# theislab/dca

Measured on NVIDIA H100. Metric: cells/sec (ZINB AE epoch, device-timed), higher is better.
Workload: dtype bf16-gemm/f32-acc/f32-loss

## Files before the change

### dca_b200/csrc/dense_tc.cu

```cuda
#include <mutex>
#include "engine.h"
#include "tc_common.cuh"
#include "head_act.cuh"

namespace dca {
namespace tc {

typedef CUresult (*EncodeTiledFn)(CUtensorMap*, CUtensorMapDataType, cuuint32_t, void*, const cuuint64_t*,
                                  const cuuint64_t*, const cuuint32_t*, const cuuint32_t*, CUtensorMapInterleave,
                                  CUtensorMapSwizzle, CUtensorMapL2promotion, CUtensorMapFloatOOBfill);

static EncodeTiledFn encode_fn() {
  static EncodeTiledFn fn = nullptr;
  static std::once_flag once;
  std::call_once(once, [] {
    void* p = nullptr;
    cudaDriverEntryPointQueryResult q;
    if (cudaGetDriverEntryPoint("cuTensorMapEncodeTiled", &p, cudaEnableDefault, &q) == cudaSuccess &&
        q == cudaDriverEntryPointSuccess)
      fn = reinterpret_cast<EncodeTiledFn>(p);
  });
  return fn;
}

int make_tensor_map_2d(CUtensorMap* out, const void* base, int elem_bytes, int is_bf16, uint64_t rows, uint64_t cols,
                       uint64_t ld_elems, uint32_t box_rows, uint32_t box_cols, int swizzle) {
  EncodeTiledFn fn = encode_fn();
  if (!fn) { set_error("cuTensorMapEncodeTiled is not available from the driver"); return DCA_ERR_CUDA; }
  cuuint64_t dims[2] = {cols, rows};
  cuuint64_t strides[1] = {ld_elems * (uint64_t)elem_bytes};
  cuuint32_t box[2] = {box_cols, box_rows};
  cuuint32_t estr[2] = {1, 1};
  const CUtensorMapDataType dt = is_bf16 ? CU_TENSOR_MAP_DATA_TYPE_BFLOAT16 : CU_TENSOR_MAP_DATA_TYPE_FLOAT32;
  CUresult r = fn(out, dt, 2, const_cast<void*>(base), dims, strides, box, estr, CU_TENSOR_MAP_INTERLEAVE_NONE,
                  swizzle ? CU_TENSOR_MAP_SWIZZLE_128B : CU_TENSOR_MAP_SWIZZLE_NONE, CU_TENSOR_MAP_L2_PROMOTION_L2_256B,
                  CU_TENSOR_MAP_FLOAT_OOB_FILL_NONE);
  if (r != CUDA_SUCCESS) {
    set_error("cuTensorMapEncodeTiled failed (%d): rows=%llu cols=%llu ld=%llu box=%ux%u elem=%d", (int)r,
              (unsigned long long)rows, (unsigned long long)cols, (unsigned long long)ld_elems, box_rows, box_cols, elem_bytes);
    return DCA_ERR_CUDA;
  }
  return DCA_OK;
}

struct ProbeParams {
  int a_mn, b_mn, M, N, K;
  int a_boxes, a_box_bytes, a_box_c0, a_box_c1;
  int b_boxes, b_box_bytes, b_box_c0, b_box_c1;
  uint32_t a_lbo, a_sbo, a_kstep, a_kblock_steps, a_kblock_bytes, a_mn64_bytes;
  uint32_t b_lbo, b_sbo, b_kstep, b_kblock_steps, b_kblock_bytes, b_mn64_bytes;
};

template <int NC, int TA, int TB>
__device__ __forceinline__ void probe_mma(float (&acc)[NC / 2], uint64_t da, uint64_t db) {
  if constexpr (NC == 128) wgmma_m64n128k16<TA, TB>(acc, da, db, 1u);
  else wgmma_m64n64k16<TA, TB>(acc, da, db, 1u);
}

template <int NC>
__device__ __forceinline__ void probe_chunk(const ProbeParams& p, uint32_t sa, uint32_t sb, int m0, int n0, float* D) {
  float acc[NC / 2];
#pragma unroll
  for (int i = 0; i < NC / 2; ++i) acc[i] = 0.f;
  const uint32_t a0 = sa + (uint32_t)(m0 / 64) * p.a_mn64_bytes, b0 = sb + (uint32_t)(n0 / 64) * p.b_mn64_bytes;
  wgmma_fence();
  for (int j = 0; j < p.K / 16; ++j) {
    const uint32_t aoff = (j / p.a_kblock_steps) * p.a_kblock_bytes + (j % p.a_kblock_steps) * p.a_kstep;
    const uint32_t boff = (j / p.b_kblock_steps) * p.b_kblock_bytes + (j % p.b_kblock_steps) * p.b_kstep;
    const uint64_t da = make_smem_desc(a0 + aoff, p.a_lbo, p.a_sbo), db = make_smem_desc(b0 + boff, p.b_lbo, p.b_sbo);
    if (p.a_mn) { if (p.b_mn) probe_mma<NC, 1, 1>(acc, da, db); else probe_mma<NC, 1, 0>(acc, da, db); }
    else        { if (p.b_mn) probe_mma<NC, 0, 1>(acc, da, db); else probe_mma<NC, 0, 0>(acc, da, db); }
  }
  wgmma_commit();
  wgmma_wait<0>();
  acc_fence(acc);
  const int w = threadIdx.x >> 5, l = threadIdx.x & 31;
#pragma unroll
  for (int i = 0; i < NC / 2; ++i) {
    const int row = m0 + 16 * w + (l >> 2) + 8 * ((i >> 1) & 1), col = n0 + 8 * (i >> 2) + 2 * (l & 3) + (i & 1);
    D[(size_t)row * p.N + col] = acc[i];
  }
}

__global__ void __launch_bounds__(128, 1)
tc_probe_kernel(const __grid_constant__ CUtensorMap map_a, const __grid_constant__ CUtensorMap map_b,
                const ProbeParams p, float* __restrict__ D) {
  extern __shared__ __align__(1024) uint8_t smem_raw[];
  uint8_t* smem = smem_raw + ((1024u - (smem_u32(smem_raw) & 1023u)) & 1023u);
  __shared__ uint64_t bar_load;
  uint8_t* sa = smem;
  uint8_t* sb = smem + (size_t)p.a_boxes * p.a_box_bytes;
  if (threadIdx.x == 0) { mbar_init(&bar_load, 1); fence_barrier_init(); }
  __syncthreads();
  if (threadIdx.x == 0) {
    mbar_expect_tx(&bar_load, (uint32_t)(p.a_boxes * p.a_box_bytes + p.b_boxes * p.b_box_bytes));
    for (int i = 0; i < p.a_boxes; ++i) tma_load_2d(sa + (size_t)i * p.a_box_bytes, &map_a, i * p.a_box_c0, i * p.a_box_c1, &bar_load);
    for (int i = 0; i < p.b_boxes; ++i) tma_load_2d(sb + (size_t)i * p.b_box_bytes, &map_b, i * p.b_box_c0, i * p.b_box_c1, &bar_load);
  }
  mbar_wait(&bar_load, 0);
  for (int m0 = 0; m0 < p.M; m0 += 64)
    for (int n0 = 0; n0 < p.N;) {
      if (p.N - n0 >= 128) { probe_chunk<128>(p, smem_u32(sa), smem_u32(sb), m0, n0, D); n0 += 128; }
      else { probe_chunk<64>(p, smem_u32(sa), smem_u32(sb), m0, n0, D); n0 += 64; }
    }
}

namespace k2 {
constexpr int BM = 128, BN = 128, BK = 64;
constexpr int kThreads = 256;
constexpr uint32_t kABytes = BM * BK * 2, kBBytes = BN * BK * 2;
constexpr uint32_t kSmemBytes = kABytes + kBBytes + 1024;

struct Params {
  int B, G, n_heads;
  int kind[3];
  int m_tiles, n_tiles_per_head;
  const float* bias[3];
  const float* row_scale;
  float* out[3]; int64_t ld_out;
};

__global__ void __launch_bounds__(kThreads, 2)
heads_fwd_kernel(const __grid_constant__ CUtensorMap map_h, const __grid_constant__ CUtensorMap map_w0,
                 const __grid_constant__ CUtensorMap map_w1, const __grid_constant__ CUtensorMap map_w2, const Params p) {
  extern __shared__ __align__(1024) uint8_t smem_raw[];
  uint8_t* smem = smem_raw + ((1024u - (smem_u32(smem_raw) & 1023u)) & 1023u);
  __shared__ uint64_t full_bar;
  const int mt = blockIdx.x % p.m_tiles, r = blockIdx.x / p.m_tiles;
  const int nt = r % p.n_tiles_per_head, hs = r / p.n_tiles_per_head;
  if (threadIdx.x == 0) {
    mbar_init(&full_bar, 1);
    fence_barrier_init();
    const CUtensorMap* mw = hs == 0 ? &map_w0 : (hs == 1 ? &map_w1 : &map_w2);
    mbar_expect_tx(&full_bar, kABytes + kBBytes);
    tma_load_2d(smem, &map_h, 0, mt * BM, &full_bar);
    tma_load_2d(smem + kABytes, mw, nt * BN, 0, &full_bar);
    tma_load_2d(smem + kABytes + kBBytes / 2, mw, nt * BN + 64, 0, &full_bar);
  }
  __syncthreads();
  const int wg = threadIdx.x >> 7, w = (threadIdx.x >> 5) & 3, l = threadIdx.x & 31;
  const int col0 = nt * BN + 2 * (l & 3);
  const int row0 = mt * BM + wg * 64 + 16 * w + (l >> 2);
  const float* bias = p.bias[hs];
  const int kind = p.kind[hs];
  float2 bz[16];
#pragma unroll
  for (int c = 0; c < 16; ++c) bz[c] = (col0 + 8 * c < p.G) ? *reinterpret_cast<const float2*>(bias + col0 + 8 * c) : make_float2(0.f, 0.f);
  float rs[2] = {1.f, 1.f};
  if (kind == EPI_MEAN_ACT && p.row_scale) {
    if (row0 < p.B) rs[0] = p.row_scale[row0];
    if (row0 + 8 < p.B) rs[1] = p.row_scale[row0 + 8];
  }
  float acc[64];
#pragma unroll
  for (int i = 0; i < 64; ++i) acc[i] = 0.f;
  mbar_wait(&full_bar, 0);
  head_tile_mma(acc, smem_u32(smem) + wg * 64 * 128, smem_u32(smem) + kABytes);
  float* out = p.out[hs];
  auto emit = [&](auto act) {
#pragma unroll
    for (int h = 0; h < 2; ++h) {
      const int row = row0 + 8 * h;
      if (row >= p.B) continue;
      float* orow = out + (int64_t)row * p.ld_out;
#pragma unroll
      for (int c = 0; c < 16; ++c) {
        const int col = col0 + 8 * c;
        if (col < p.G)
          *reinterpret_cast<float2*>(orow + col) =
              make_float2(act(acc[4 * c + 2 * h], bz[c].x, rs[h]), act(acc[4 * c + 2 * h + 1], bz[c].y, rs[h]));
      }
    }
  };
  if (kind == EPI_MEAN_ACT) emit([](float a, float b, float s) { return head_out<EPI_MEAN_ACT>(a, b, s); });
  else if (kind == EPI_DISP_ACT) emit([](float a, float b, float s) { return head_out<EPI_DISP_ACT>(a, b, s); });
  else emit([](float a, float b, float s) { return head_out<EPI_SIGMOID>(a, b, s); });
}
}

int heads_fwd_tc(const __nv_bfloat16* Hb, int B, const __nv_bfloat16* const W[3], const float* const bias[3], int G,
                 int n_heads, const int kind[3], const float* row_scale, float* const out[3], int64_t ld_out, int sm_count,
                 cudaStream_t s) {
  using namespace k2;
  if (ld_out % 4 != 0 || G % 8 != 0) { set_error("heads_fwd_tc: G must be a multiple of 8 and ld_out of 4 (TMA strides)"); return DCA_ERR_BAD_ARG; }
  CUtensorMap mh, mw[3];
  DCA_TRY(make_tensor_map_2d(&mh, Hb, 2, 1, (uint64_t)B, 64, 64, BM, BK, 1));
  for (int i = 0; i < 3; ++i)
    DCA_TRY(make_tensor_map_2d(&mw[i], W[i < n_heads ? i : 0], 2, 1, 64, (uint64_t)G, (uint64_t)G, 64, 64, 1));
  Params p;
  p.B = B; p.G = G; p.n_heads = n_heads;
  for (int i = 0; i < 3; ++i) { const int k = i < n_heads ? i : 0; p.kind[i] = kind[i]; p.bias[i] = bias[k]; p.out[i] = out[k]; }
  p.m_tiles = cdiv(B, BM); p.n_tiles_per_head = cdiv(G, BN);
  p.row_scale = row_scale; p.ld_out = ld_out;
  (void)sm_count;
  static bool attr_set = false;
  if (!attr_set) {
    DCA_CUDA_OK(cudaFuncSetAttribute(heads_fwd_kernel, cudaFuncAttributeMaxDynamicSharedMemorySize, (int)kSmemBytes));
    attr_set = true;
  }
  const int grid = p.m_tiles * p.n_tiles_per_head * n_heads;
  heads_fwd_kernel<<<grid, kThreads, kSmemBytes, s>>>(mh, mw[0], mw[1], mw[2], p);
  DCA_LAUNCH_CHECK();
  return DCA_OK;
}

}

Engine::~Engine() {
  comm_destroy();
  for (auto e : prof.ev) cudaEventDestroy(e);
  for (auto& g : graphs) if (g.exec) cudaGraphExecDestroy(g.exec);
  if (hs.copy) cudaStreamDestroy(hs.copy);
  if (hs.expand) cudaStreamDestroy(hs.expand);
  for (int k = 0; k < 3; ++k) {
    if (hs.ready[k]) cudaEventDestroy(hs.ready[k]);
    if (hs.step_done[k]) cudaEventDestroy(hs.step_done[k]);
  }
  for (int k = 0; k < 2; ++k) {
    if (hs.h2d_done[k]) cudaEventDestroy(hs.h2d_done[k]);
    if (hs.cnt_free[k]) cudaEventDestroy(hs.cnt_free[k]);
  }
}

}

using namespace dca;

extern "C" int dca_tc_probe(const void* A, int32_t a_rows, int32_t a_cols, const void* Bm, int32_t b_rows, int32_t b_cols,
                            int32_t a_mn_major, int32_t b_mn_major, int32_t M, int32_t N, int32_t K,
                            int32_t a_lbo, int32_t a_sbo, int32_t b_lbo, int32_t b_sbo, float* D, void* stream) {
  using namespace tc;
  if (M != 128 || N % 64 != 0 || N < 64 || N > 256 || K % 64 != 0 || K <= 0 || K > 256) {
    set_error("dca_tc_probe: need M=128, N%%64==0 (64..256), K%%64==0 (<=256)"); return DCA_ERR_BAD_ARG;
  }
  ProbeParams p{};
  p.a_mn = a_mn_major; p.b_mn = b_mn_major; p.M = M; p.N = N; p.K = K;
  CUtensorMap ma, mb;
  auto setup = [&](int mn, int mn_extent, int rows, int cols, const void* base, CUtensorMap* map, int& boxes, int& box_bytes,
                   int& c0, int& c1, uint32_t& lbo, uint32_t& sbo, uint32_t& kstep, uint32_t& kb_steps, uint32_t& kb_bytes,
                   uint32_t& mn64_bytes, int lbo_o, int sbo_o) -> int {
    if (!mn) {
      if (rows != mn_extent || cols != K) { set_error("dca_tc_probe: K-major operand must be [MN x K]"); return DCA_ERR_BAD_ARG; }
      DCA_TRY(make_tensor_map_2d(map, base, 2, 1, rows, cols, cols, mn_extent, 64, 1));
      boxes = K / 64; box_bytes = mn_extent * 128; c0 = 64; c1 = 0;
      lbo = 0; sbo = 1024; kstep = 32; kb_steps = 4; kb_bytes = box_bytes; mn64_bytes = 64 * 128;
    } else {
      if (rows != K || cols != mn_extent || mn_extent % 64) { set_error("dca_tc_probe: MN-major operand must be [K x MN], MN%%64==0"); return DCA_ERR_BAD_ARG; }
      DCA_TRY(make_tensor_map_2d(map, base, 2, 1, rows, cols, cols, K, 64, 1));
      boxes = mn_extent / 64; box_bytes = K * 128; c0 = 64; c1 = 0;
      lbo = box_bytes; sbo = 1024; kstep = 2048; kb_steps = 1u << 30; kb_bytes = 0; mn64_bytes = box_bytes;
    }
    if (lbo_o >= 0) lbo = lbo_o;
    if (sbo_o >= 0) sbo = sbo_o;
    return DCA_OK;
  };
  DCA_TRY(setup(a_mn_major, M, a_rows, a_cols, A, &ma, p.a_boxes, p.a_box_bytes, p.a_box_c0, p.a_box_c1, p.a_lbo, p.a_sbo,
                p.a_kstep, p.a_kblock_steps, p.a_kblock_bytes, p.a_mn64_bytes, a_lbo, a_sbo));
  DCA_TRY(setup(b_mn_major, N, b_rows, b_cols, Bm, &mb, p.b_boxes, p.b_box_bytes, p.b_box_c0, p.b_box_c1, p.b_lbo, p.b_sbo,
                p.b_kstep, p.b_kblock_steps, p.b_kblock_bytes, p.b_mn64_bytes, b_lbo, b_sbo));
  const size_t smem = (size_t)p.a_boxes * p.a_box_bytes + (size_t)p.b_boxes * p.b_box_bytes + 1024;
  DCA_CUDA_OK(cudaFuncSetAttribute(tc_probe_kernel, cudaFuncAttributeMaxDynamicSharedMemorySize, (int)smem));
  tc_probe_kernel<<<1, 128, smem, (cudaStream_t)stream>>>(ma, mb, p, D);
  DCA_LAUNCH_CHECK();
  return DCA_OK;
}

extern "C" int dca_tc_heads_fwd(const void* Hb, int32_t batch, const void* Wk, const float* bias, int32_t genes,
                                int32_t n_heads, const int32_t kind[3], const float* row_scale, float* out0, float* out1,
                                float* out2, int64_t ld_out, void* stream) {
  if (!Hb || !Wk || !bias || batch <= 0 || genes <= 0 || n_heads < 1 || n_heads > 3 || !out0) {
    set_error("dca_tc_heads_fwd: bad argument"); return DCA_ERR_BAD_ARG;
  }
  int dev = 0, sms = 132;
  cudaGetDevice(&dev);
  cudaDeviceGetAttribute(&sms, cudaDevAttrMultiProcessorCount, dev);
  int k[3] = {kind[0], n_heads > 1 ? kind[1] : 0, n_heads > 2 ? kind[2] : 0};
  float* outs[3] = {out0, out1, out2};
  const __nv_bfloat16* W[3]; const float* b[3];
  for (int i = 0; i < 3; ++i) {
    const int j = i < n_heads ? i : 0;
    W[i] = (const __nv_bfloat16*)Wk + (size_t)j * 64 * genes; b[i] = bias + (size_t)j * genes;
  }
  return tc::heads_fwd_tc((const __nv_bfloat16*)Hb, batch, W, b, genes, n_heads, k, row_scale, outs, ld_out, sms,
                          (cudaStream_t)stream);
}
```

### dca_b200/csrc/head_act.cuh

```cuda
#pragma once
#include "dca_internal.cuh"
#include "tc_common.cuh"

namespace dca {
namespace tc {

__device__ __forceinline__ float act_mean(float z) { return fminf(fmaxf(ex2f(z * 1.442695041f), 1e-5f), 1e6f); }
__device__ __forceinline__ float act_disp(float z) {
  const float e = ex2f(-fabsf(z) * 1.442695041f);
  const float l_series = e * fmaf(e, fmaf(e, 0.333333333f, -0.5f), 1.0f);
  const float l_log = 0.693147181f * lg2f(1.0f + e);
  const float sp = fmaxf(z, 0.f) + (e < 0.01f ? l_series : l_log);
  return fminf(fmaxf(sp, 1e-4f), 1e4f);
}
__device__ __forceinline__ float act_sigmoid(float z) { return rcpf(1.0f + ex2f(-z * 1.442695041f)); }

__device__ __forceinline__ void head_tile_mma(float (&acc)[64], uint32_t h_smem, uint32_t w_smem) {
  wgmma_fence();
#pragma unroll
  for (int k = 0; k < 4; ++k)
    wgmma_m64n128k16<0, 1>(acc, make_smem_desc(h_smem + k * 32, 0, 1024), make_smem_desc(w_smem + k * 2048, 8192, 1024), k > 0);
  wgmma_commit();
  wgmma_wait<0>();
  acc_fence(acc);
}

template <int KIND>
__device__ __forceinline__ float head_out(float acc, float bias, float row_scale) {
  const float z = acc + bias;
  if (KIND == EPI_MEAN_ACT) return act_mean(z) * row_scale;
  if (KIND == EPI_DISP_ACT) return act_disp(z);
  return act_sigmoid(z);
}

}
}
```

### dca_b200/csrc/zinb_loss.cu

```cuda
#include "dca_internal.cuh"
#include <string>
#include "zinb_math.cuh"
#include "tc_common.cuh"
#include "head_act.cuh"
#include <cstdlib>

namespace dca {
namespace tc { extern int g_gg_profile; }

namespace {

constexpr int kThreads = 256;
constexpr int kVec = 4;
constexpr int kColsPerBlock = kThreads * kVec;
constexpr int kMaxBlocks = 65536;

struct LossTune { int target_blocks; unsigned producer_sleep_ns, consumer_sleep_ns; int branch_free; int ring; };
LossTune g_tune = {0 , 0u, 0u, 1 ,
                   1 };

int sm_count_cached() {
  static int n = 0;
  if (!n) { int dev = 0; if (cudaGetDevice(&dev) != cudaSuccess || cudaDeviceGetAttribute(&n, cudaDevAttrMultiProcessorCount, dev) != cudaSuccess || n <= 0) n = 132; }
  return n;
// ... 595 lines not shown
  }
  __syncthreads();

  const uint32_t my = tc::smem_u32(smem_ring) + threadIdx.x * 16;
  const uint32_t ring_end = my + RING * kSlotBytes;
  const float* ysrc = Y + c0 + col;
  const float* msrc = m + (int64_t)r0 * ld + c0 + col;
  const float* dsrc = COND_DISP ? d + (int64_t)r0 * ld + c0 + col : nullptr;
  const float* psrc = pi + (int64_t)r0 * ld + c0 + col;
  const uint32_t ldy32 = (uint32_t)ldy;
  int nxt = 0;
  uint32_t wslot = my;
  auto cp16 = [](uint32_t dst, const void* src) {
    asm volatile("cp.async.cg.shared.global [%0], [%1], 16;" ::"r"(dst), "l"(src) : "memory");
  };
  auto issue_next = [&]() {
    cp16(wslot, ysrc + (uint64_t)((uint32_t)s_row[nxt]) * ldy32);
    cp16(wslot + kSegBytes, msrc);
    if (COND_DISP) cp16(wslot + 2 * kSegBytes, dsrc);
    cp16(wslot + (kArrays - 1) * kSegBytes, psrc);
    msrc += ld; psrc += ld;
    if (COND_DISP) dsrc += ld;
    ++nxt; wslot += kSlotBytes;
    if (wslot == ring_end) wslot = my;
  };

  float lsum_lg = 0.f, lsum_nb = 0.f, lsum_r = 0.f;
  float tacc[kVec] = {0.f, 0.f, 0.f, 0.f};
  {
#pragma unroll
    for (int i = 0; i < RING; ++i) {
      if (i < nrows) issue_next();
      cp_async_commit();
    }
    float4* q = items + warp * (32 * kVec);
    unsigned char* qb = reinterpret_cast<unsigned char*>(items) + warp * (32 * kVec);
    auto lds32 = [](uint32_t addr) { float v; asm volatile("ld.shared.f32 %0, [%1];" : "=f"(v) : "r"(addr) : "memory"); return v; };
    auto sts32 = [](uint32_t addr, float v) { asm volatile("st.shared.f32 [%0], %1;" ::"r"(addr), "f"(v) : "memory"); };
    float thg[kVec] = {1.f, 1.f, 1.f, 1.f};
    if (!COND_DISP) {
#pragma unroll
      for (int j = 0; j < kVec; ++j) thg[j] = d[c0 + col + j];
    }
    const unsigned lt = (1u << lane) - 1u;
    GT* om = dzm + (int64_t)r0 * ld + c0 + col;
    GT* od = COND_DISP ? dzd + (int64_t)r0 * ld + c0 + col : nullptr;
    GT* op = dzp + (int64_t)r0 * ld + c0 + col;
    uint32_t rslot = my;
    auto lds128 = [](uint32_t addr) {
      float4 v;
      asm volatile("ld.shared.v4.f32 {%0,%1,%2,%3}, [%4];" : "=f"(v.x), "=f"(v.y), "=f"(v.z), "=f"(v.w) : "r"(addr) : "memory");
      return v;
    };
    for (int i = 0; i < nrows; ++i) {
      cp_async_wait<RING - 1>();
      const uint32_t cslot = rslot, wstrip = rslot - (uint32_t)lane * 16u;
      const float4 vy = lds128(rslot), vm = lds128(rslot + kSegBytes);
      const float4 vd = COND_DISP ? lds128(rslot + 2 * kSegBytes) : make_float4(thg[0], thg[1], thg[2], thg[3]);
      const float4 vp = lds128(rslot + (kArrays - 1) * kSegBytes);
      rslot += kSlotBytes;
      if (rslot == ring_end) rslot = my;
      const float row_sf = s_sf[i];
      if constexpr (!IDXQ) {
        const RowGrads g = zinb_row_ring<COND_DISP>(vy, vm, vd, vp, row_sf, active, ridge, inv_n, q, lf, lsum_lg, lsum_nb,
                                                    lsum_r, tacc, [&] { if (nxt < nrows) issue_next(); cp_async_commit(); });
        if (active) {
          st4(om, g.gmA.x, g.gmA.y, g.gmB.x, g.gmB.y);
          if (COND_DISP) st4(od, g.gdA.x, g.gdA.y, g.gdB.x, g.gdB.y);
          st4(op, g.gpA.x, g.gpA.y, g.gpB.x, g.gpB.y);
        }
      } else {
      const float y[kVec] = {vy.x, vy.y, vy.z, vy.w};
      const float2 mA = make_float2(vm.x, vm.y), mB = make_float2(vm.z, vm.w);
      const float2 dA = make_float2(vd.x, vd.y), dB = make_float2(vd.z, vd.w);
      const float2 pA = make_float2(vp.x, vp.y), pB = make_float2(vp.z, vp.w);
      const float2 muA = mul2(mA, splat(row_sf)), muB = mul2(mB, splat(row_sf));
      const float dd[kVec] = {dA.x, dA.y, dB.x, dB.y};
      bool isnz[kVec];
      int pos[kVec], base = 0;
#pragma unroll
      for (int j = 0; j < kVec; ++j) {
        isnz[j] = active && !(y[j] < 1e-8f);
        const unsigned bal = __ballot_sync(kFull, isnz[j]);
        pos[j] = base + __popc(bal & lt); base += __popc(bal);
      }
      const int total = base;
#pragma unroll
      for (int j = 0; j < kVec; ++j)
        if (isnz[j]) qb[pos[j]] = (unsigned char)(lane * kVec + j);
      __syncwarp();
      const float m_lo = fminf(fminf(vm.x, vm.y), fminf(vm.z, vm.w)), m_hi = fmaxf(fmaxf(vm.x, vm.y), fmaxf(vm.z, vm.w));
      const float d_lo = fminf(fminf(dd[0], dd[1]), fminf(dd[2], dd[3])), d_hi = fmaxf(fmaxf(dd[0], dd[1]), fmaxf(dd[2], dd[3]));
      const bool plain = (m_lo > 1e-5f) && (m_hi < 1e6f) &&
                         (COND_DISP ? (d_lo > 0.03125f) && (d_hi < 1e4f) : (d_hi <= 1e6f));
      Raw2 zA, zB; Fin2 fA, fB;
      if (__all_sync(kFull, plain)) {
        zA = zinb_zero_pair<Ops, true>(muA, dA, pA); zB = zinb_zero_pair<Ops, true>(muB, dB, pB);
        fA = finish_factors_pair_plain<Ops, COND_DISP>(dA, pA, inv_n); fB = finish_factors_pair_plain<Ops, COND_DISP>(dB, pB, inv_n);
      } else {
        zA = zinb_zero_pair<Ops>(muA, dA, pA); zB = zinb_zero_pair<Ops>(muB, dB, pB);
        fA = finish_factors_pair<Ops, COND_DISP>(mA, dA, pA, inv_n); fB = finish_factors_pair<Ops, COND_DISP>(mB, dB, pB, inv_n);
      }
      lsum_lg += ((active && !isnz[0]) ? zA.lgD.x : 0.f) + ((active && !isnz[1]) ? zA.lgD.y : 0.f)
               + ((active && !isnz[2]) ? zB.lgD.x : 0.f) + ((active && !isnz[3]) ? zB.lgD.y : 0.f);
      for (int k = lane; k < total; k += 32) {
        const int idx = qb[k];
        const uint32_t e4 = wstrip + (uint32_t)idx * 4u;
        const float th = COND_DISP ? lds32(e4 + 2 * kSegBytes) : __ldg(d + c0 + warp * (32 * kVec) + idx);
        const Raw1 e = zinb_nb_raw<Ops>(lds32(e4), lds32(e4 + kSegBytes) * row_sf, th, lds32(e4 + (kArrays - 1) * kSegBytes), lf);
        lsum_nb += e.loss;
        sts32(e4, e.gmu); sts32(e4 + kSegBytes, e.dth); sts32(e4 + (kArrays - 1) * kSegBytes, e.dpi);
      }
      __syncwarp();
      const float4 r0v = lds128(cslot), r1v = lds128(cslot + kSegBytes), r2v = lds128(cslot + (kArrays - 1) * kSegBytes);
      zA.gmu.x = isnz[0] ? r0v.x : zA.gmu.x; zA.dth.x = isnz[0] ? r1v.x : zA.dth.x; zA.dpi.x = isnz[0] ? r2v.x : zA.dpi.x;
      zA.gmu.y = isnz[1] ? r0v.y : zA.gmu.y; zA.dth.y = isnz[1] ? r1v.y : zA.dth.y; zA.dpi.y = isnz[1] ? r2v.y : zA.dpi.y;
      zB.gmu.x = isnz[2] ? r0v.z : zB.gmu.x; zB.dth.x = isnz[2] ? r1v.z : zB.dth.x; zB.dpi.x = isnz[2] ? r2v.z : zB.dpi.x;
      zB.gmu.y = isnz[3] ? r0v.w : zB.gmu.y; zB.dth.y = isnz[3] ? r1v.w : zB.dth.y; zB.dpi.y = isnz[3] ? r2v.w : zB.dpi.y;
      __syncwarp();
      if (nxt < nrows) issue_next();
      cp_async_commit();
      if (ridge != 0.f) {
        if (active) lsum_r += ridge * (pA.x * pA.x + pA.y * pA.y + pB.x * pB.x + pB.y * pB.y);
        zA.dpi = fma2(splat(2.0f * ridge), pA, zA.dpi); zB.dpi = fma2(splat(2.0f * ridge), pB, zB.dpi);
      }
      if (active) {
        if (!COND_DISP) { tacc[0] += zA.dth.x; tacc[1] += zA.dth.y; tacc[2] += zB.dth.x; tacc[3] += zB.dth.y; }
        const float2 gmA = mul2(zA.gmu, fA.fm), gmB = mul2(zB.gmu, fB.fm);
        const float2 gpA = mul2(zA.dpi, fA.fp), gpB = mul2(zB.dpi, fB.fp);
        st4(om, gmA.x, gmA.y, gmB.x, gmB.y);
        if (COND_DISP) {
          const float2 gdA = mul2(zA.dth, fA.fd), gdB = mul2(zB.dth, fB.fd);
          st4(od, gdA.x, gdA.y, gdB.x, gdB.y);
        }
        st4(op, gpA.x, gpA.y, gpB.x, gpB.y);
      }
      }
      om += ld; op += ld;
      if (COND_DISP) od += ld;
    }
    if (!COND_DISP && active) {
#pragma unroll
      for (int j = 0; j < kVec; ++j) atomicAdd(dth_acc + c0 + col + j, tacc[j]);
    }
  }
  block_loss_fold<kThreads>((double)lsum_nb + (double)lsum_r - (double)kLn2 * (double)lsum_lg,
                            red, &s_last, loss_partial, fa, inv_n);
}

namespace hl {
constexpr int kWG = 4;
constexpr int kCtaThreads = 128 * kWG;
constexpr int kRows = 4;
constexpr int kPieces = 16 / kRows;
constexpr uint32_t kWHeadBytes = 64 * 128 * 2;
constexpr uint32_t kHBytes = 64 * 64 * 2;
constexpr uint32_t kRowBytes = 3 * 128 * 4;
constexpr uint32_t kQPad = 512;
constexpr uint32_t kOffY = kQPad + kRows * kRowBytes;
constexpr uint32_t kWarpBytes = kOffY + kRows * 128 * 4;
constexpr uint32_t kOffH = 3 * kWHeadBytes;
constexpr uint32_t kOffStage = kOffH + kWG * kHBytes;
constexpr uint32_t kOffBias = kOffStage + kWG * 4 * kWarpBytes;
constexpr uint32_t kSmemBytes = kOffBias + 3 * 128 * 4 + 1024;
static_assert(kSmemBytes + 1024 <= 227 * 1024, "heads_loss_kernel: dynamic + 1 KB static shared memory over the sm_90 limit");

struct Params {
  const float* bias[3];
  const float* Y; int64_t ldy; const int32_t* rows; const float* sf;
  int B, G, nblk, units;
  float ridge, inv_n;
  __nv_bfloat16* dz[3]; int64_t ldz;
  double* loss_partial; const float* lf;
};

__device__ __forceinline__ uint32_t slot16(int i, int k) { return (uint32_t)((i ^ ((2 * k) & 6)) * 16); }

__device__ __forceinline__ void stage_acc(const float (&acc)[64], int piece, uint8_t* head_base) {
  const int lane = threadIdx.x & 31, k = (lane >> 2) & 3;
  if ((lane >> 4) != (piece & 1)) return;
  const bool hi = piece >= 2;
  uint8_t* dst = head_base + k * kRowBytes + (lane & 1) * 8;
#pragma unroll
  for (int c = 0; c < 16; ++c) {
    const int g = 8 * c + 2 * (lane & 3);
    *reinterpret_cast<float2*>(dst + slot16(g >> 2, k)) =
        make_float2(hi ? acc[4 * c + 2] : acc[4 * c], hi ? acc[4 * c + 3] : acc[4 * c + 1]);
  }
}

template <int KIND>
__device__ __forceinline__ float4 head_out4(const float4 a, const float4 b) {
  return make_float4(tc::head_out<KIND>(a.x, b.x, 1.0f), tc::head_out<KIND>(a.y, b.y, 1.0f),
                     tc::head_out<KIND>(a.z, b.z, 1.0f), tc::head_out<KIND>(a.w, b.w, 1.0f));
}
}

__global__ void __launch_bounds__(hl::kCtaThreads, 1)
heads_loss_kernel(const __grid_constant__ CUtensorMap map_h, const __grid_constant__ CUtensorMap map_w0,
                  const __grid_constant__ CUtensorMap map_w1, const __grid_constant__ CUtensorMap map_w2, const hl::Params p,
                  const FoldArgs fa) {
  using namespace hl;
  using namespace tc;
  extern __shared__ __align__(1024) uint8_t smem_hl_raw[];
  uint8_t* smem = smem_hl_raw + ((1024u - (smem_u32(smem_hl_raw) & 1023u)) & 1023u);
  __shared__ uint64_t w_bar, h_bar[kWG];
  __shared__ float lf[zmath::kLogFactN];
  __shared__ double red[kCtaThreads / 32];
  __shared__ int s_last;
  const int tid = threadIdx.x, wg = tid >> 7, warp = (tid >> 5) & 3, lane = tid & 31;
  float* s_bias = reinterpret_cast<float*>(smem + kOffBias);
  uint8_t* h_buf = smem + kOffH + wg * kHBytes;
  uint8_t* wbase = smem + kOffStage + (wg * 4 + warp) * kWarpBytes;
  uint8_t* rows_base = wbase + kQPad;
  const uint32_t my_y = smem_u32(wbase + kOffY) + lane * 16;
  if (tid < zmath::kLogFactN) lf[tid] = p.lf[tid];
  if (tid == 0) {
    mbar_init(&w_bar, 1);
    for (int g = 0; g < kWG; ++g) mbar_init(&h_bar[g], 1);
    fence_barrier_init();
  }
  __syncthreads();
  const CUtensorMap* mw[3] = {&map_w0, &map_w1, &map_w2};
  auto load_h = [&](int blk) {
    if ((tid & 127) == 0) { mbar_expect_tx(&h_bar[wg], kHBytes); tma_load_2d(h_buf, &map_h, 0, blk * 64, &h_bar[wg]); }
  };
  const int u0 = (int)((long long)blockIdx.x * p.units / gridDim.x), u1 = (int)((long long)(blockIdx.x + 1) * p.units / gridDim.x);
  uint32_t w_phase = 0, h_phase = 0;
  float lsum_lg = 0.f, lsum_nb = 0.f, lsum_r = 0.f;
  float tacc[kVec] = {0.f, 0.f, 0.f, 0.f};
  for (int u = u0; u < u1;) {
    const int t = u / p.nblk;
    const int seg_end = min(u1, (t + 1) * p.nblk);
    const int b_end = seg_end - t * p.nblk;
    int blk = u - t * p.nblk + wg;
    __syncthreads();
    if (tid == 0) {
      mbar_expect_tx(&w_bar, 3 * kWHeadBytes);
      for (int h = 0; h < 3; ++h) {
        tma_load_2d(smem + h * kWHeadBytes, mw[h], t * 128, 0, &w_bar);
        tma_load_2d(smem + h * kWHeadBytes + kWHeadBytes / 2, mw[h], t * 128 + 64, 0, &w_bar);
      }
    }
    if (tid < 3 * 128) {
      const int gcol = t * 128 + (tid & 127);
      const float* bias = wg == 0 ? p.bias[0] : (wg == 1 ? p.bias[1] : p.bias[2]);
      s_bias[tid] = gcol < p.G ? bias[gcol] : 0.f;
    }
    if (blk < b_end) load_h(blk);
    __syncthreads();
    mbar_wait(&w_bar, w_phase); w_phase ^= 1;
    const int gvalid = min(128, p.G - t * 128);
    const bool active = 4 * lane < gvalid;
    const int col = active ? 4 * lane : gvalid - kVec;
    const int64_t gcol0 = (int64_t)t * 128 + col;
    for (; blk < b_end; blk += kWG) {
      mbar_wait(&h_bar[wg], h_phase); h_phase ^= 1;
      for (int piece = 0; piece < kPieces; ++piece) {
        const int r0 = blk * 64 + warp * 16 + piece * kRows;
        int my_yr = 0; float my_sf = 1.f;
        if (lane < kRows && r0 + lane < p.B) {
          my_yr = p.rows ? p.rows[r0 + lane] : r0 + lane;
          my_sf = p.sf ? p.sf[my_yr] : 1.0f;
        }
        float acc[64];
        head_tile_mma(acc, smem_u32(h_buf), smem_u32(smem));
        stage_acc(acc, piece, rows_base);
#pragma unroll
        for (int k = 0; k < kRows; ++k) {
          const int yr = __shfl_sync(0xffffffffu, my_yr, k);
          if (r0 + k < p.B)
            asm volatile("cp.async.cg.shared.global [%0], [%1], 16;" ::"r"(my_y + k * 512), "l"(p.Y + (int64_t)yr * p.ldy + gcol0)
                         : "memory");
        }
        cp_async_commit();
        head_tile_mma(acc, smem_u32(h_buf), smem_u32(smem) + kWHeadBytes);
        stage_acc(acc, piece, rows_base + 512);
        head_tile_mma(acc, smem_u32(h_buf), smem_u32(smem) + 2 * kWHeadBytes);
        if (piece == kPieces - 1) {
          named_barrier_sync(1 + wg, 128);
          if (blk + kWG < b_end) load_h(blk + kWG);
        }
        stage_acc(acc, piece, rows_base + 1024);
        cp_async_wait<0>();
        __syncwarp();
        for (int k = 0; k < kRows; ++k) {
          const int r = r0 + k;
          if (r >= p.B) break;
          float4 vy;
          asm volatile("ld.shared.v4.f32 {%0,%1,%2,%3}, [%4];" : "=f"(vy.x), "=f"(vy.y), "=f"(vy.z), "=f"(vy.w) : "r"(my_y + k * 512)
                       : "memory");
          const float row_sf = __shfl_sync(0xffffffffu, my_sf, k);
          const uint8_t* src = rows_base + k * kRowBytes + slot16(col >> 2, k);
          const float4 am = *reinterpret_cast<const float4*>(src);
          const float4 ad = *reinterpret_cast<const float4*>(src + 512);
          const float4 ap = *reinterpret_cast<const float4*>(src + 1024);
          __syncwarp();
          const float4 vm = head_out4<EPI_MEAN_ACT>(am, *reinterpret_cast<const float4*>(s_bias + col));
          const float4 vd = head_out4<EPI_DISP_ACT>(ad, *reinterpret_cast<const float4*>(s_bias + 128 + col));
          const float4 vp = head_out4<EPI_SIGMOID>(ap, *reinterpret_cast<const float4*>(s_bias + 256 + col));
          float4* q = reinterpret_cast<float4*>(wbase + k * kRowBytes);
          const RowGrads g = zinb_row_ring<true>(vy, vm, vd, vp, row_sf, active, p.ridge, p.inv_n, q, lf, lsum_lg, lsum_nb,
                                                 lsum_r, tacc, [] {});
          if (active) {
            const int64_t off = (int64_t)r * p.ldz + gcol0;
            st4(p.dz[0] + off, g.gmA.x, g.gmA.y, g.gmB.x, g.gmB.y);
            st4(p.dz[1] + off, g.gdA.x, g.gdA.y, g.gdB.x, g.gdB.y);
            st4(p.dz[2] + off, g.gpA.x, g.gpA.y, g.gpB.x, g.gpB.y);
          }
        }
      }
    }
    u = seg_end;
  }
  block_loss_fold<kCtaThreads>((double)lsum_nb + (double)lsum_r - (double)zmath::kLn2 * (double)lsum_lg, red, &s_last,
                            p.loss_partial, fa, p.inv_n);
}

__global__ void fold_partials_kernel(const double* __restrict__ part, int n, double* out, int accumulate,
                                     const double* penalty, float inv_n, int batch, float* loss_slot, double* epoch_acc) {
  __shared__ double sm[32];
  double a = 0.0;
  for (int i = threadIdx.x; i < n; i += blockDim.x) a += part[i];
#pragma unroll
  for (int o = 16; o > 0; o >>= 1) a += __shfl_xor_sync(0xffffffffu, a, o);
  if ((threadIdx.x & 31) == 0) sm[threadIdx.x >> 5] = a;
  __syncthreads();
  if (threadIdx.x < 32) {
    a = (threadIdx.x < (blockDim.x >> 5)) ? sm[threadIdx.x] : 0.0;
#pragma unroll
    for (int o = 16; o > 0; o >>= 1) a += __shfl_xor_sync(0xffffffffu, a, o);
    if (threadIdx.x == 0) {
      *out = accumulate ? (*out + a) : a;
      if (loss_slot) {
        double l = a * (double)inv_n;
        if (l != l) l = INFINITY;
        if (penalty) l += *penalty;
        const float lf = (float)l;
        loss_slot[0] = lf;
        loss_slot[1] = (isfinite(lf)) ? 0.f : 1.f;
        if (epoch_acc) { epoch_acc[0] += l * (double)batch; epoch_acc[1] += (double)batch; }
      }
    }
  }
}

__device__ float g_log_fact[zmath::kLogFactN];

const float* log_fact_table_device() {
  static thread_local int ready_dev = -1;
  static thread_local float* cached = nullptr;
  int dev = 0;
  if (cudaGetDevice(&dev) != cudaSuccess) { set_error("cudaGetDevice failed"); return nullptr; }
  if (ready_dev == dev && cached) return cached;
  float* p = nullptr;
  if (cudaGetSymbolAddress((void**)&p, g_log_fact) != cudaSuccess) { set_error("cudaGetSymbolAddress failed"); return nullptr; }
  cached = p;
  if (ready_dev != dev) {
    float t[zmath::kLogFactN];
    zmath::fill_log_fact(t);
    if (cudaMemcpy(p, t, sizeof(t), cudaMemcpyHostToDevice) != cudaSuccess) { set_error("log-factorial table upload failed"); return nullptr; }
    ready_dev = dev;
  }
  return p;
}

template <bool BWD>
int launch(const LossArgs& a, cudaStream_t s) {
  if (a.B <= 0 || a.G <= 0) { set_error("zinb_loss: empty batch (B=%d, G=%d)", a.B, a.G); return DCA_ERR_BAD_ARG; }
  const bool has_pi = (a.ae_type == DCA_AE_ZINB_CONDDISP || a.ae_type == DCA_AE_ZINB);
  const bool cond = (a.ae_type == DCA_AE_ZINB_CONDDISP || a.ae_type == DCA_AE_NB_CONDDISP);
  if (!a.Y || !a.m || !a.d || (has_pi && !a.pi) || !a.loss_sum) { set_error("zinb_loss: null input"); return DCA_ERR_BAD_ARG; }
  if (BWD && (!a.dzm || (cond && !a.dzd) || (has_pi && !a.dzp) || (!cond && !a.dtheta))) {
    set_error("zinb_loss: null gradient output"); return DCA_ERR_BAD_ARG;
  }
  const float* lf_dev = log_fact_table_device();
  if (!lf_dev) return DCA_ERR_CUDA;
  const size_t need = loss_workspace_bytes(a.B, a.G);
  if (!a.ws || a.ws_bytes < need) { set_error("zinb_loss: workspace too small (%zu < %zu)", a.ws_bytes, need); return DCA_ERR_BAD_ARG; }
  double* lpart = reinterpret_cast<double*>(a.ws);
  auto al16 = [](const void* q) { return (reinterpret_cast<uintptr_t>(q) & 15) == 0; };
  bool vec = (a.G % 4 == 0) && (a.ld % 4 == 0) && (a.ldy % 4 == 0) && al16(a.Y) && al16(a.m) && (!cond || al16(a.d)) &&
             (!has_pi || al16(a.pi));
  if (BWD) vec = vec && al16(a.dzm) && (!cond || al16(a.dzd)) && (!has_pi || al16(a.dzp));
  const Plan p = make_plan(a.B, a.G, vec ? kColsPerBlock : kThreads);
  dim3 grid(p.col_blocks, p.row_chunks), block(kThreads);
  float* tpart = a.dtheta;
  if (BWD && !cond) DCA_CUDA_OK(cudaMemsetAsync(a.dtheta, 0, sizeof(float) * (size_t)a.G, s));

  static const bool use_compact = [] { const char* e = getenv("DCA_LOSS_KERNEL"); return e && e[0] == 'c'; }();
  const Plan ps = make_plan(a.B, a.G, kColsPerBlock, kMaxRowsPerBlock);
  const bool staged_ok = BWD && vec && has_pi && !use_compact && (long long)ps.row_chunks * ps.col_blocks <= kMaxBlocks &&
                         ps.row_chunks <= 65535;
  if (staged_ok) {
    grid = dim3(ps.col_blocks, ps.row_chunks);
    FoldArgs fa{reinterpret_cast<unsigned*>(reinterpret_cast<char*>(a.ws) + sizeof(double) * (size_t)kMaxBlocks), a.loss_sum,
                a.fin_penalty, a.fin_loss_slot, a.fin_epoch_acc, a.fin_batch};
    if (!a.counter_ready) DCA_CUDA_OK(cudaMemsetAsync(fa.counter, 0, sizeof(unsigned), s));
#define DCA_RING2(CD, GT, IQ)                                                                                     \
  do {                                                                                                             \
    constexpr size_t sm = IQ ? (size_t)(kRing + 1) * (CD ? 4 : 3) * kColsPerBlock * 4 + (size_t)(kThreads / 32) * 32 * kVec     \
                             : (size_t)kRing * (CD ? 4 : 3) * kColsPerBlock * 4 + (size_t)(kThreads / 32) * 32 * kVec * 16; \
    static bool attr = false;                                                                                      \
    if (!attr) { DCA_CUDA_OK(cudaFuncSetAttribute(zinb_loss_bwd_ring_kernel<CD, GT, IQ>, cudaFuncAttributeMaxDynamicSharedMemorySize, (int)sm)); attr = true; } \
    zinb_loss_bwd_ring_kernel<CD, GT, IQ><<<grid, kThreads, sm, s>>>(a.Y, a.ldy, a.rows, a.sf, a.m, a.d, a.pi, a.ld, a.B, a.G, a.ridge, \
        a.inv_n, ps.rows_per_block, (GT*)a.dzm, (GT*)a.dzd, (GT*)a.dzp, tpart, lpart, lf_dev, fa);                  \
  } while (0)
#define DCA_RING(CD, GT) do { if (g_tune.ring == 2) DCA_RING2(CD, GT, true); else DCA_RING2(CD, GT, false); } while (0)
    if (g_tune.ring) {
      if (a.grad_bf16) { if (cond) DCA_RING(true, __nv_bfloat16); else DCA_RING(false, __nv_bfloat16); }
      else             { if (cond) DCA_RING(true, float); else DCA_RING(false, float); }
      DCA_LAUNCH_CHECK();
      return DCA_OK;
    }
#undef DCA_RING
#undef DCA_RING2
#define DCA_STAGED2(CD, GT, BFV)                                                                                   \
  do {                                                                                                             \
    constexpr size_t sm = (size_t)kStageRows * (CD ? 4 : 3) * kColsPerBlock * 4 + (size_t)(kThreads / 32) * 32 * kVec * 16; \
    static bool attr = false;                                                                                      \
    if (!attr) { DCA_CUDA_OK(cudaFuncSetAttribute(zinb_loss_bwd_staged_kernel<CD, GT, BFV>, cudaFuncAttributeMaxDynamicSharedMemorySize, (int)sm)); attr = true; } \
    zinb_loss_bwd_staged_kernel<CD, GT, BFV><<<grid, kStagedThreads, sm, s>>>(a.Y, a.ldy, a.rows, a.sf, a.m, a.d, a.pi, a.ld, a.B, \
        a.G, a.ridge, a.inv_n, ps.rows_per_block, (GT*)a.dzm, (GT*)a.dzd, (GT*)a.dzp, tpart, lpart, lf_dev, fa,     \
        g_tune.producer_sleep_ns, g_tune.consumer_sleep_ns);                                                       \
  } while (0)
#define DCA_STAGED(CD, GT) do { if (g_tune.branch_free) DCA_STAGED2(CD, GT, true); else DCA_STAGED2(CD, GT, false); } while (0)
    if (a.grad_bf16) { if (cond) DCA_STAGED(true, __nv_bfloat16); else DCA_STAGED(false, __nv_bfloat16); }
    else             { if (cond) DCA_STAGED(true, float); else DCA_STAGED(false, float); }
#undef DCA_STAGED2
#undef DCA_STAGED
    DCA_LAUNCH_CHECK();
    return DCA_OK;
  } else if (BWD && vec && has_pi) {
#define DCA_COMPACT(CD, GT)                                                                                   \
  zinb_loss_bwd_compact_kernel<CD, GT><<<grid, block, 0, s>>>(a.Y, a.ldy, a.rows, a.sf, a.m, a.d, a.pi, a.ld, a.B, a.G, \
                                                              a.ridge, a.inv_n, p.rows_per_block, (GT*)a.dzm,  \
// ... 191 lines not shown
```

Measured before the change: 2.678 million.

## Compute ZINB head outputs per 16-cell piece with transposed n16 wgmma

```diff
diff --git a/dca_b200/csrc/dense_tc.cu b/dca_b200/csrc/dense_tc.cu
--- a/dca_b200/csrc/dense_tc.cu
+++ b/dca_b200/csrc/dense_tc.cu
@@ -54,7 +54,8 @@
 template <int NC, int TA, int TB>
 __device__ __forceinline__ void probe_mma(float (&acc)[NC / 2], uint64_t da, uint64_t db) {
   if constexpr (NC == 128) wgmma_m64n128k16<TA, TB>(acc, da, db, 1u);
-  else wgmma_m64n64k16<TA, TB>(acc, da, db, 1u);
+  else if constexpr (NC == 64) wgmma_m64n64k16<TA, TB>(acc, da, db, 1u);
+  else wgmma_m64n16k16<TA, TB>(acc, da, db, 1u);
 }
 
 template <int NC>
@@ -100,7 +101,8 @@
   mbar_wait(&bar_load, 0);
   for (int m0 = 0; m0 < p.M; m0 += 64)
     for (int n0 = 0; n0 < p.N;) {
-      if (p.N - n0 >= 128) { probe_chunk<128>(p, smem_u32(sa), smem_u32(sb), m0, n0, D); n0 += 128; }
+      if (p.N == 16) { probe_chunk<16>(p, smem_u32(sa), smem_u32(sb), m0, n0, D); n0 += 16; }
+      else if (p.N - n0 >= 128) { probe_chunk<128>(p, smem_u32(sa), smem_u32(sb), m0, n0, D); n0 += 128; }
       else { probe_chunk<64>(p, smem_u32(sa), smem_u32(sb), m0, n0, D); n0 += 64; }
     }
 }
@@ -230,8 +232,8 @@
                             int32_t a_mn_major, int32_t b_mn_major, int32_t M, int32_t N, int32_t K,
                             int32_t a_lbo, int32_t a_sbo, int32_t b_lbo, int32_t b_sbo, float* D, void* stream) {
   using namespace tc;
-  if (M != 128 || N % 64 != 0 || N < 64 || N > 256 || K % 64 != 0 || K <= 0 || K > 256) {
-    set_error("dca_tc_probe: need M=128, N%%64==0 (64..256), K%%64==0 (<=256)"); return DCA_ERR_BAD_ARG;
+  if (M != 128 || (N != 16 && (N % 64 != 0 || N < 64 || N > 256)) || K % 64 != 0 || K <= 0 || K > 256) {
+    set_error("dca_tc_probe: need M=128, N=16 or N%%64==0 (64..256), K%%64==0 (<=256)"); return DCA_ERR_BAD_ARG;
   }
   ProbeParams p{};
   p.a_mn = a_mn_major; p.b_mn = b_mn_major; p.M = M; p.N = N; p.K = K;
diff --git a/dca_b200/csrc/head_act.cuh b/dca_b200/csrc/head_act.cuh
--- a/dca_b200/csrc/head_act.cuh
+++ b/dca_b200/csrc/head_act.cuh
@@ -25,6 +25,17 @@
   acc_fence(acc);
 }
 
+__device__ __forceinline__ void head_piece_mma(float (&acc)[2][8], uint32_t h_smem, uint32_t w_smem) {
+  wgmma_fence();
+#pragma unroll
+  for (int mb = 0; mb < 2; ++mb)
+#pragma unroll
+    for (int k = 0; k < 4; ++k)
+      wgmma_m64n16k16<1, 0>(acc[mb], make_smem_desc(w_smem + mb * 8192 + k * 2048, 8192, 1024),
+                            make_smem_desc(h_smem + k * 32, 0, 1024), k > 0);
+  wgmma_commit();
+}
+
 template <int KIND>
 __device__ __forceinline__ float head_out(float acc, float bias, float row_scale) {
   const float z = acc + bias;
diff --git a/dca_b200/csrc/zinb_loss.cu b/dca_b200/csrc/zinb_loss.cu
--- a/dca_b200/csrc/zinb_loss.cu
+++ b/dca_b200/csrc/zinb_loss.cu
@@ -771,13 +771,15 @@
 constexpr int kWG = 4;
 constexpr int kCtaThreads = 128 * kWG;
 constexpr int kRows = 4;
-constexpr int kPieces = 16 / kRows;
+constexpr int kPieceCells = 4 * kRows;
+constexpr int kPieces = 64 / kPieceCells;
 constexpr uint32_t kWHeadBytes = 64 * 128 * 2;
 constexpr uint32_t kHBytes = 64 * 64 * 2;
 constexpr uint32_t kRowBytes = 3 * 128 * 4;
 constexpr uint32_t kQPad = 512;
 constexpr uint32_t kOffY = kQPad + kRows * kRowBytes;
-constexpr uint32_t kWarpBytes = kOffY + kRows * 128 * 4;
+constexpr uint32_t kWarpBytes = kOffY + kRows * 128 * 4 + 32;
+static_assert(kWarpBytes % 128 == 32, "stage_head's stores are conflict-free only with warp areas 32 B apart modulo 128 B");
 constexpr uint32_t kOffH = 3 * kWHeadBytes;
 constexpr uint32_t kOffStage = kOffH + kWG * kHBytes;
 constexpr uint32_t kOffBias = kOffStage + kWG * 4 * kWarpBytes;
@@ -795,17 +797,16 @@
 
 __device__ __forceinline__ uint32_t slot16(int i, int k) { return (uint32_t)((i ^ ((2 * k) & 6)) * 16); }
 
-__device__ __forceinline__ void stage_acc(const float (&acc)[64], int piece, uint8_t* head_base) {
-  const int lane = threadIdx.x & 31, k = (lane >> 2) & 3;
-  if ((lane >> 4) != (piece & 1)) return;
-  const bool hi = piece >= 2;
-  uint8_t* dst = head_base + k * kRowBytes + (lane & 1) * 8;
-#pragma unroll
-  for (int c = 0; c < 16; ++c) {
-    const int g = 8 * c + 2 * (lane & 3);
-    *reinterpret_cast<float2*>(dst + slot16(g >> 2, k)) =
-        make_float2(hi ? acc[4 * c + 2] : acc[4 * c], hi ? acc[4 * c + 3] : acc[4 * c + 1]);
-  }
+__device__ __forceinline__ void stage_head(const float (&acc)[2][8], uint8_t* wg_stage, int h) {
+  const int warp = (threadIdx.x >> 5) & 3, lane = threadIdx.x & 31;
+  uint8_t* base = wg_stage + ((lane >> 1) & 1) * kWarpBytes + kQPad + 2 * (lane & 1) * kRowBytes + h * 512 + ((lane >> 2) & 3) * 4 +
+                  ((((4 * warp) ^ (4 * (lane & 1))) | (lane >> 4)) * 16);
+#pragma unroll
+  for (int mb = 0; mb < 2; ++mb)
+#pragma unroll
+    for (int i = 0; i < 8; ++i)
+      *reinterpret_cast<float*>(base + 2 * (i >> 2) * kWarpBytes + (i & 1) * kRowBytes + (16 * mb | (2 * (((i >> 1) ^ i) & 1))) * 16) =
+          acc[mb][i];
 }
 
 template <int KIND>
@@ -830,7 +831,8 @@
   const int tid = threadIdx.x, wg = tid >> 7, warp = (tid >> 5) & 3, lane = tid & 31;
   float* s_bias = reinterpret_cast<float*>(smem + kOffBias);
   uint8_t* h_buf = smem + kOffH + wg * kHBytes;
-  uint8_t* wbase = smem + kOffStage + (wg * 4 + warp) * kWarpBytes;
+  uint8_t* wg_stage = smem + kOffStage + wg * 4 * kWarpBytes;
+  uint8_t* wbase = wg_stage + warp * kWarpBytes;
   uint8_t* rows_base = wbase + kQPad;
   const uint32_t my_y = smem_u32(wbase + kOffY) + lane * 16;
   if (tid < zmath::kLogFactN) lf[tid] = p.lf[tid];
@@ -875,16 +877,19 @@
     const int64_t gcol0 = (int64_t)t * 128 + col;
     for (; blk < b_end; blk += kWG) {
       mbar_wait(&h_bar[wg], h_phase); h_phase ^= 1;
-      for (int piece = 0; piece < kPieces; ++piece) {
-        const int r0 = blk * 64 + warp * 16 + piece * kRows;
+      const int last_piece = min(kPieces, (p.B - blk * 64 + kPieceCells - 1) / kPieceCells) - 1;
+      for (int piece = 0; piece <= last_piece; ++piece) {
+        float acc[3][2][8];
+        const uint32_t h_piece = smem_u32(h_buf) + piece * kPieceCells * 128;
+        head_piece_mma(acc[0], h_piece, smem_u32(smem));
+        head_piece_mma(acc[1], h_piece, smem_u32(smem) + kWHeadBytes);
+        head_piece_mma(acc[2], h_piece, smem_u32(smem) + 2 * kWHeadBytes);
+        const int r0 = blk * 64 + piece * kPieceCells + warp * kRows;
         int my_yr = 0; float my_sf = 1.f;
         if (lane < kRows && r0 + lane < p.B) {
           my_yr = p.rows ? p.rows[r0 + lane] : r0 + lane;
           my_sf = p.sf ? p.sf[my_yr] : 1.0f;
         }
-        float acc[64];
-        head_tile_mma(acc, smem_u32(h_buf), smem_u32(smem));
-        stage_acc(acc, piece, rows_base);
 #pragma unroll
         for (int k = 0; k < kRows; ++k) {
           const int yr = __shfl_sync(0xffffffffu, my_yr, k);
@@ -893,14 +898,15 @@
                          : "memory");
         }
         cp_async_commit();
-        head_tile_mma(acc, smem_u32(h_buf), smem_u32(smem) + kWHeadBytes);
-        stage_acc(acc, piece, rows_base + 512);
-        head_tile_mma(acc, smem_u32(h_buf), smem_u32(smem) + 2 * kWHeadBytes);
-        if (piece == kPieces - 1) {
-          named_barrier_sync(1 + wg, 128);
-          if (blk + kWG < b_end) load_h(blk + kWG);
-        }
-        stage_acc(acc, piece, rows_base + 1024);
+        named_barrier_sync(1 + wg, 128);
+        wgmma_wait<2>(); acc_fence(acc[0][0]); acc_fence(acc[0][1]);
+        stage_head(acc[0], wg_stage, 0);
+        wgmma_wait<1>(); acc_fence(acc[1][0]); acc_fence(acc[1][1]);
+        stage_head(acc[1], wg_stage, 1);
+        wgmma_wait<0>(); acc_fence(acc[2][0]); acc_fence(acc[2][1]);
+        stage_head(acc[2], wg_stage, 2);
+        named_barrier_sync(1 + wg, 128);
+        if (piece == last_piece && blk + kWG < b_end) load_h(blk + kWG);
         cp_async_wait<0>();
         __syncwarp();
         for (int k = 0; k < kRows; ++k) {
```

New measurement: 2.809 million (median of 6 runs). 4.9% higher.
